# aromanro/DFTAtom

Measured on AMD Instinct MI355X. Metric: numerov_sweeps_per_s (executed sweeps of the reference's bisection path, whole SCF step; Rn Z=86 @ 131073 pts), higher is better.
Workload: dtype f64

## Files before the change

### dftatom_amd/__init__.py

```python
import ctypes as C
import os

import numpy as np

_HERE = os.path.dirname(os.path.abspath(__file__))
LIB_PATH = os.environ.get("DFTA_LIB_PATH") or os.path.join(_HERE, "libdftatom_hip.so")

OK = 0
SWEEP_COUNT, SWEEP_ZERO = 0, 1
SWEEP_KERNEL_AUTO, SWEEP_KERNEL_FUSED, SWEEP_KERNEL_PIPELINED = 0, 1, 2
BOUNDARY_DEVICE, BOUNDARY_HOST = 0, 1
LEVELS_CHAINED, LEVELS_BATCHED = 0, 1
LEVELS_SCAN_SWEEPS = 0x10
SWEEPS_EXACT, SWEEPS_TOLERANCE = 0, 1
ABI_VERSION = 7
LEVEL_CONVERGED, LEVEL_ITERATION_CAP, LEVEL_FIXED_POINT, LEVEL_U0_NONFINITE = 1, 2, 4, 8
POISSON_DEFAULT, POISSON_EXACT, POISSON_TOLERANCE, POISSON_ADAPTIVE = -1, 0, 1, 2
INT_TRAPEZOID, INT_SIMPSON13, INT_SIMPSON38, INT_BOOLE, INT_ROMBERG = range(5)
XC_VWN, XC_CHACHIYO, XC_CHACHIYO_IMPROVED, XC_PW92, XC_PBE = range(5)
AUFBAU_REFERENCE, AUFBAU_TRANSITION_METALS = range(2)
MIX_LINEAR, MIX_ANDERSON = range(2)
RECORD_DOUBLES = 64
ORB_PROPS = 8
ORB_NORM, ORB_RM1, ORB_R1, ORB_R2, ORB_R4, ORB_T, ORB_RPEAK, ORB_RM3 = range(8)
# ... 52 lines not shown
    "dfta_grid_destroy": (None, [vp]),
    "dfta_grid_num_nodes": (C.c_int, [vp]),
    "dfta_grid_rp": (C.c_double, [vp]),
    "dfta_grid_get_r": (C.c_int, [vp, c_dp]),
    "dfta_num_nodes": (C.c_int, [C.c_int]),
    "dfta_numerov_sweeps": (C.c_int, [vp, vp, C.c_int, C.c_int, C.c_int, c_dp, C.c_int, c_ip, c_ip, c_dp, c_ip,
                                      c_ip, c_dp, c_ip, c_ip]),
    "dfta_numerov_sweeps_scan": (C.c_int, [vp, vp, C.c_int, C.c_int, c_dp, C.c_int, c_ip, c_ip, c_dp, c_ip, c_ip, c_dp, c_ip, c_ip, c_ip]),
    "dfta_numerov_sweeps_dev": (C.c_int, [vp, vp, C.c_int, C.c_int, vp, C.c_int, c_ip, c_ip, c_ip, vp, vp, vp, vp, vp,
                                          vp, vp, vp, vp]),
    "dfta_numerov_match": (C.c_int, [vp, vp, C.c_int, C.c_int, c_dp, C.c_int, c_ip, c_ip, c_dp, c_dp, c_lp]),
    "dfta_potential_create": (C.c_int, [vp, vp, c_dp, C.POINTER(vp)]),
    "dfta_potential_update": (C.c_int, [vp, c_dp]),
    "dfta_potential_destroy": (None, [vp]),
    "dfta_potential_sweeps": (C.c_int, [vp, C.c_int, C.c_int, C.c_int, c_ip, c_dp, c_ip, c_ip, c_dp, c_ip, c_ip]),
    "dfta_potential_match": (C.c_int, [vp, C.c_int, c_ip, c_dp, c_dp, c_lp]),
    "dfta_solve_levels": (C.c_int, [vp, vp, C.c_int, C.c_int, C.c_int, c_dp, c_dp, c_dp, C.c_int, c_ip, c_ip, c_ip, c_ip,
                                    C.POINTER(LevelResult), c_dp, c_dp, c_dp, c_lp]),
    "dfta_poisson_create": (C.c_int, [vp, vp, C.c_int, C.POINTER(vp)]),
    "dfta_poisson_destroy": (None, [vp]),
    "dfta_poisson_solve": (C.c_int, [vp, c_ip, c_dp, c_dp, c_ip, c_dp]),
    "dfta_poisson_solve_dev": (C.c_int, [vp, vp, vp, vp]),
    "dfta_poisson_group_info": (C.c_int, [vp, c_ip, c_ip, c_ip]),
    "dfta_scf_poisson_info": (C.c_int, [vp, c_ip, c_ip, c_ip]),
    "dfta_poisson_level_size": (C.c_int, [vp, C.c_int]),
    "dfta_poisson_set_level": (C.c_int, [vp, C.c_int, c_dp, c_dp]),
    "dfta_poisson_get_level": (C.c_int, [vp, C.c_int, c_dp, c_dp]),
    "dfta_poisson_gauss_seidel": (C.c_int, [vp, C.c_int, C.c_int, c_dp]),
    "dfta_poisson_iterate_gs": (C.c_int, [vp, C.c_int, C.c_double, C.c_int, C.POINTER(C.c_double), C.POINTER(C.c_int)]),
    "dfta_poisson_restrict": (C.c_int, [vp, C.c_int]),
    "dfta_poisson_prolong": (C.c_int, [vp, C.c_int]),
    "dfta_poisson_vcycle": (C.c_int, [vp, c_dp]),
    "dfta_poisson_full_cycle": (C.c_int, [vp, C.c_double, C.c_double, C.c_double, C.c_double, c_dp, c_ip]),
    "dfta_scf_set_integrator": (C.c_int, [vp, C.c_int]),
    "dfta_vwn_lda": (C.c_int, [vp, c_dp, C.c_size_t, c_dp, c_dp]),
    "dfta_vwn_lsda": (C.c_int, [vp, c_dp, c_dp, C.c_size_t, c_dp, c_dp, c_dp, c_dp]),
    "dfta_integrate": (C.c_int, [vp, C.c_int, C.c_double, c_dp, C.c_int, C.POINTER(C.c_double)]),
    "dfta_scf_create": (C.c_int, [vp, vp, C.c_int, C.c_int, c_ip, C.c_double, C.c_int, C.c_int, C.POINTER(vp)]),
    "dfta_scf_create_ex": (C.c_int, [vp, vp, C.c_int, C.c_int, c_ip, C.c_double, C.c_int, C.c_int, vp, C.POINTER(vp)]),
    "dfta_scf_destroy": (None, [vp]),
    "dfta_scf_step": (C.c_int, [vp, C.POINTER(StepStats)]),
    "dfta_scf_get_energies": (C.c_int, [vp, C.POINTER(Energies), c_ip]),
    "dfta_scf_info": (C.c_int, [vp, c_ip, c_ip, c_lp]),
    "dfta_scf_num_levels": (C.c_int, [vp, C.c_int, C.c_int]),
    "dfta_scf_get_levels": (C.c_int, [vp, C.c_int, C.c_int, c_ip, c_ip, c_ip, c_dp, c_ip]),
    "dfta_scf_get_level_status": (C.c_int, [vp, C.c_int, C.c_int, c_ip, c_ip, c_ip]),
# ... 291 lines not shown
        self.ctx, self.grid, self.batch = ctx, grid, batch
        h = vp()
        if mode == POISSON_DEFAULT:
            ctx.check(ctx.lib.dfta_poisson_create(ctx.h, grid.h, batch, C.byref(h)))
        else:
            ctx.check(ctx.lib.dfta_poisson_create_ex(ctx.h, grid.h, batch, int(mode), C.byref(h)))
        self.h = h
        self.mode = ctx.lib.dfta_poisson_mode(h)

    def solve(self, Z, density):
        Z = _i32(np.atleast_1d(Z))
        rho = _f64(density).reshape(self.batch, self.grid.N)
        U = np.zeros_like(rho)
        vc = np.zeros(self.batch, np.int32)
        err = np.zeros(self.batch)
        self.ctx.check(self.ctx.lib.dfta_poisson_solve(self.h, _ip(Z), _dp(rho), _dp(U), _ip(vc), _dp(err)))
        return U, vc, err

    def group_info(self):
        g, d, a = C.c_int(), C.c_int(), C.c_int()
        self.ctx.check(self.ctx.lib.dfta_poisson_group_info(self.h, C.byref(g), C.byref(d), C.byref(a)))
        return g.value, bool(d.value), a.value

    def level_size(self, lvl):
        return self.ctx.lib.dfta_poisson_level_size(self.h, lvl)

    def set_level(self, lvl, phi=None, src=None):
        self.ctx.check(self.ctx.lib.dfta_poisson_set_level(self.h, lvl, _dp(_f64(phi)) if phi is not None else None,
                                                           _dp(_f64(src)) if src is not None else None))

    def get_level(self, lvl):
        n = self.level_size(lvl)
        phi, src = np.zeros(n), np.zeros(n)
        self.ctx.check(self.ctx.lib.dfta_poisson_get_level(self.h, lvl, _dp(phi), _dp(src)))
        return phi, src

    def gauss_seidel(self, lvl, sweeps=1):
        err = np.zeros(sweeps)
        self.ctx.check(self.ctx.lib.dfta_poisson_gauss_seidel(self.h, lvl, sweeps, _dp(err)))
        return err

    def iterate_gs(self, lvl, error_min, iterno):
        err = C.c_double()
        n = C.c_int()
        self.ctx.check(self.ctx.lib.dfta_poisson_iterate_gs(self.h, lvl, error_min, iterno, C.byref(err), C.byref(n)))
        return err.value, n.value
# ... 288 lines not shown
```

### dftatom_amd/csrc/poisson.hip

```cpp
#include <hip/hip_runtime.h>

#include <algorithm>
#include <cmath>
#include <cstdlib>
#include <memory>
#include <type_traits>
#include <vector>

#include "internal.h"
#include "poisson_plan.h"
#include "xc.h"

using namespace dfta_mg;

namespace {

#ifndef DFTA_KWARM
#define DFTA_KWARM 96
#endif
constexpr int kPF = 8;

__host__ __device__ __forceinline__ int addr(const Lvl& L, int i)
{
    if (i == L.n - 1) return L.n - 1;
// ... 168 lines not shown
    ++p->aborts;
    DFTA_HIP(ctx, hipMemsetAsync(p->d_total_vcycles, 0, sizeof(unsigned long long), ctx->stream));
    int rc = degrade(p);
    if (rc) return rc;
    rc = dfta_poisson_solve_launch(p->fallback.get(), dNe, dDensity, dU, dVcycles, dErr, dSkip);
    if (rc) return rc;
    DFTA_HIP(ctx, hipStreamSynchronize(ctx->stream));
    return DFTA_OK;
}

int dfta_poisson_take_vcycles(dfta_poisson* p, unsigned long long* out)
{
    dfta_ctx* ctx = p->ctx;
    unsigned long long a = 0, b = 0;
    DFTA_HIP(ctx, hipMemcpyAsync(&a, p->d_total_vcycles, sizeof(unsigned long long), hipMemcpyDeviceToHost, ctx->stream));
    if (p->fallback) DFTA_HIP(ctx, hipMemcpyAsync(&b, p->fallback->d_total_vcycles, sizeof(unsigned long long), hipMemcpyDeviceToHost, ctx->stream));
    DFTA_HIP(ctx, hipStreamSynchronize(ctx->stream));
    DFTA_HIP(ctx, hipMemsetAsync(p->d_total_vcycles, 0, sizeof(unsigned long long), ctx->stream));
    if (p->fallback) DFTA_HIP(ctx, hipMemsetAsync(p->fallback->d_total_vcycles, 0, sizeof(unsigned long long), ctx->stream));
    *out = a + b;
    return DFTA_OK;
}

int dfta_poisson_group_state(const dfta_poisson* p, int* G, int* degraded, int* aborts)
{
    if (!p) return DFTA_ERR_INVALID;
    if (G) *G = p->resident ? p->res_wg() : p->D.G;
    if (degraded) *degraded = p->degraded ? 1 : 0;
    if (aborts) *aborts = p->aborts;
    return DFTA_OK;
}

extern "C" {

int dfta_poisson_create_ex(dfta_ctx* ctx, const dfta_grid* g, int batch, int mode, dfta_poisson** out)
{
    if (!ctx || !g || !out) return DFTA_ERR_INVALID;
    DFTA_ENTER(ctx);
    DFTA_REQUIRE(ctx, mode == DFTA_POISSON_EXACT || mode == DFTA_POISSON_TOLERANCE || mode == DFTA_POISSON_ADAPTIVE, "poisson mode");
    return poisson_create_impl(ctx, g, batch, -1, mode, out);
}

int dfta_poisson_create(dfta_ctx* ctx, const dfta_grid* g, int batch, dfta_poisson** out)
{
    if (!ctx || !g || !out) return DFTA_ERR_INVALID;
    DFTA_ENTER(ctx);
// ... 9 lines not shown
    auto set = [](const char* value) { return value != nullptr; };
    auto on_off = [](const char* value) { return value ? (atoi(value) != 0 ? 1 : 0) : -1; };
    PoissonKnobs K;
    if (const char* e = dfta_knob("POISSON_GROUP")) {
        const int v = atoi(e);
        K.group_set = true;
        if (v >= 0 && v <= 6 && (batch << v) <= 256) K.group = v;
    }
    if (const char* e = dfta_knob("FAULT_POISSON_MEMBER")) K.fault = atoi(e) != 0;
    K.res = on_off(dfta_knob("POISSON_RES"));
    K.res16 = on_off(dfta_knob("POISSON_RES16"));
    K.nostage = set(dfta_knob("POISSON_NOSTAGE"));
    K.nostage_wave = set(dfta_knob("POISSON_NOSTAGE_WAVE"));
    K.nostage_shared = set(dfta_knob("POISSON_NOSTAGE_SHARED"));
    K.nocoarse = set(dfta_knob("POISSON_NOCOARSE"));
    K.noxw = set(dfta_knob("POISSON_NOXW"));
    K.norc = set(dfta_knob("POISSON_NORC"));
    K.nofuse3 = set(dfta_knob("POISSON_NOFUSE3"));
    K.nofuse3_wave = set(dfta_knob("POISSON_NOFUSE3_WAVE"));
    K.nohalf129 = set(dfta_knob("POISSON_NOHALF129"));
    K.nofold = set(dfta_knob("POISSON_NOFOLD"));
    K.nofold_lds = set(dfta_knob("POISSON_NOFOLD_LDS"));
    K.nofuse_coop = set(dfta_knob("POISSON_NOFUSE_COOP"));
    if (const char* e = dfta_knob("POISSON_FUSE_MIN_LOGC")) K.fuse_min_logc = std::max(kFuseMinLogC, atoi(e));
    if (const char* e = dfta_knob("POISSON_DBG")) K.dbg = atoi(e);
    K.plain_launch = set(dfta_knob("POISSON_PLAIN_LAUNCH")) || getenv("ROCP_TOOL_LIBRARIES") != nullptr;
    const char* m = dfta_knob("POISSON_MODE");
    K.mode = (m && m[0] == 't') ? DFTA_POISSON_TOLERANCE : ((m && m[0] == 'a') ? DFTA_POISSON_ADAPTIVE : DFTA_POISSON_EXACT);
    return K;
}

#define TRY_HIP(call) do { const hipError_t e_ = (call); if (e_ != hipSuccess) return e_; } while (0)
static hipError_t allocate(dfta_poisson* p)
{
    const PoissonPlan& P = *p;
    hipStream_t st = p->ctx->stream;
    TRY_HIP(p->d_phi0.alloc(P.n_level_store));
    TRY_HIP(p->d_phi1.alloc(P.n_level_store));
    TRY_HIP(p->d_src.alloc(P.n_level_store));
    TRY_HIP(p->d_cur.alloc(P.n_cur));
    TRY_HIP(p->d_desc.alloc(1));
    TRY_HIP(hipMemcpyAsync(p->d_desc, &p->D, sizeof(MgDesc), hipMemcpyHostToDevice, st));
    TRY_HIP(p->d_total_vcycles.alloc(1));
    TRY_HIP(p->d_group_ctr.alloc(P.n_group_ctr));
    TRY_HIP(p->d_group_part.alloc(P.n_group_part));
    TRY_HIP(p->d_res_slots.alloc(P.n_res_slots));
    TRY_HIP(p->d_res_spill.alloc(P.n_res_spill));
    TRY_HIP(hipMemsetAsync(p->d_phi0, 0, P.n_level_store * sizeof(double), st));
    TRY_HIP(hipMemsetAsync(p->d_phi1, 0, P.n_level_store * sizeof(double), st));
    TRY_HIP(hipMemsetAsync(p->d_src, 0, P.n_level_store * sizeof(double), st));
    TRY_HIP(hipMemsetAsync(p->d_cur, 0, P.n_cur * sizeof(int), st));
    TRY_HIP(hipMemsetAsync(p->d_total_vcycles, 0, sizeof(unsigned long long), st));
    return hipStreamSynchronize(st);
}
#undef TRY_HIP

static int blocks_per_cu(const void* kernel)
{
    int per_cu = 0;
    return hipOccupancyMaxActiveBlocksPerMultiprocessor(&per_cu, kernel, kThreads, 0) == hipSuccess ? per_cu : -1;
}

static int poisson_create_impl(dfta_ctx* ctx, const dfta_grid* g, int batch, int force_logG, int mode, dfta_poisson** out)
{
    DFTA_REQUIRE(ctx, batch >= 1 && g->levels <= kMaxLevels, "poisson batch/levels");
    PlanInputs in;
    in.knobs = read_knobs(batch);
    if (mode == kModeFromKnob) mode = in.knobs.mode;
    in.N = g->N; in.levels = g->levels; in.delta = g->delta; in.uniform = g->uniform;
    in.batch = batch; in.force_logG = force_logG; in.mode = mode; in.num_cu = ctx->num_cu;
    const bool tol = mode != DFTA_POISSON_EXACT;
    in.occupancy = [tol](PlanKernel k) {
        const KernelSet& K = kKernels[tol][k == kKernelSolveRes16];
        return blocks_per_cu(k == kKernelSolve ? reinterpret_cast<const void*>(K.solve) : reinterpret_cast<const void*>(K.solve_res));
    };
// ... 238 lines not shown
```

### dftatom_amd/csrc/poisson_kernels.inc

```
constexpr int kWarm = DFTA_MG_KWARM;
struct Atom {
    double* phi0;
    double* phi1;
    double* src;
    double* lds;
    double* stage;
    unsigned cur;
    int g, G;
    unsigned* ctr;
    unsigned bar;
    double* part;
    double* fslot;
    unsigned fseq;
    double* xchg;
    int pend;
    int pend_r;
    int pend_z;
    int lds_holds;
    int spin_max;
    bool gave_up;
    __device__ __forceinline__ int lane() const { return g * kThreads + static_cast<int>(threadIdx.x); }
    __device__ __forceinline__ double* cur_phi(int l, const Lvl& L) const
    {
        const unsigned c = (cur >> l) & 1u;
        return L.seq ? lds + c * kSeqCap + L.soff : (c ? phi1 : phi0) + L.off;
    }
    __device__ __forceinline__ double* other_phi(int l, const Lvl& L) const
    {
        const unsigned c = ((cur >> l) & 1u) ^ 1u;
        return L.seq ? lds + c * kSeqCap + L.soff : (c ? phi1 : phi0) + L.off;
    }
    __device__ __forceinline__ double* src_of(const Lvl& L) const { return L.seq ? lds + 2 * kSeqCap + L.soff : src + L.off; }
};

__device__ __forceinline__ void group_sync(Atom& A)
{
    if (A.G == 1) { __syncthreads(); return; }
    __syncthreads();
    ++A.bar;
    if (threadIdx.x == 0) {
        __builtin_amdgcn_fence(__ATOMIC_RELEASE, "agent");
        __hip_atomic_fetch_add(A.ctr, 1u, __ATOMIC_RELAXED, __HIP_MEMORY_SCOPE_AGENT);
        const unsigned target = A.bar * static_cast<unsigned>(A.G);
// ... 362 lines not shown
            for (int q = 0; q < kH; ++q) { bv[q] = ps[(r + kH + q) * RS]; bx[q] = pp[((r + kH + q + 1) & Cm1) * RS]; }
            __builtin_amdgcn_sched_barrier(0);
            own(ax, as, r);
            if (r + 2 * kH < C) {
#pragma unroll
                for (int q = 0; q < kH; ++q) { as[q] = ps[(r + 2 * kH + q) * RS]; ax[q] = pp[(r + 2 * kH + q + 1) * RS]; }
            }
            __builtin_amdgcn_sched_barrier(0);
            own(bx, bv, r + kH);
        }
    }
    if (lo_g == 0) pp[0] = node0;
    return err2;
}

constexpr int kWarm3 = DFTA_MG_KWARM3;
__device__ __forceinline__ double gs_point2y(double s, double y, double yp, double dh2)
{
    const double t1 = __builtin_fma(y, 0.5, s);
    const double u = yp - y;
    const double a = __builtin_fma(yp, 0.5, t1);
    return a - dh2 * u;
}
template <int LOGC, int RS, int NT, int KST, bool CAREFUL, bool RIGHT = false>
__device__ __forceinline__ void gs_lds3(const double* __restrict__ SSbase, double* __restrict__ PPbase, const int tid, const int lo_g,
                                        const bool last_lane, const double xN, const double dh, double& e1, double& e2, double& e3,
                                        const double* rightP = nullptr, const double* rightS = nullptr)
{
    constexpr int C = 1 << LOGC, Cm1 = C - 1, kH = 8, W = kWarm3;
    static_assert(C >= 4 && C <= 32 && W % (2 * kH) == 0, "fused pass: 4..32 nodes per lane");
    typedef __attribute__((address_space(3))) double lds_f64;
    typedef __attribute__((address_space(3))) const double lds_cf64;
    const bool active = tid < NT;
    lds_cf64* ps = (lds_cf64*)(SSbase) + tid;
    lds_f64* pp = (lds_f64*)(PPbase) + tid;
    asm volatile("" : "+v"(ps), "+v"(pp));
    auto off = [](int r) constexpr -> int { return (r & Cm1) * RS + (r >> LOGC); };
    const int neg_lo = -lo_g;
    const double dh2 = 0.5 * dh;
    const double Y0 = 2.0 * PPbase[0];
    double a1 = 0, a2 = 0, a3 = 0;
    double y1 = 0, y2 = 0, y3 = 0, sA = 0, sB = 0, o0 = 0, y1p = 0, y2p = 0;
    double xr0 = 0, xr1 = 0, xr2 = 0, sr0 = 0, sr1 = 0;
    double ax[kH], as[kH], bx[kH], bv[kH];
    auto load = [&](double (&X)[kH], double (&SV)[kH], const int r0) {
        const int col = r0 >> LOGC;
        if constexpr (C <= kH) {
            lds_cf64* bs = ps + col;
            lds_cf64* bp = (lds_cf64*)pp + col;
#pragma unroll
// ... 29 lines not shown
        constexpr int nq = C < kH ? C : kH;
        lds_f64* po = pp + r0 * RS;
#pragma unroll
        for (int q = 0; q < nq; ++q) {
            const double xn = (q == nq - 1) ? ((r0 + nq == C) ? xr0 : X[q]) : X[q];
            double t = gs_point2(SV[q], y1, xn, dh);
            if (CAREFUL && first && q == 0) t = (lo_g == 0) ? Y0 : t;
            { const double d = __builtin_fma(t, -0.5, o0); a1 = __builtin_fma(d, d, a1); }
            double u = gs_point2y(sA, y2, t, dh2);
            if (CAREFUL && first && q == 1) u = (lo_g == 0) ? Y0 : u;
            if (!(first && q == 0)) { const double d = y1p - u; a2 = __builtin_fma(d, d, a2); }
            double v = gs_point2y(sB, y3, u, dh2);
            if (CAREFUL && first && q == 2) v = (lo_g == 0) ? Y0 : v;
            if (!(first && q < 2)) { const double d = y2p - v; a3 = __builtin_fma(d, d, a3); }
            if (KST == 1) po[q * RS] = 0.5 * t;
            if (KST == 2 && !(first && q == 0)) po[(q - 1) * RS] = 0.5 * u;
            if (KST == 3 && !(first && q < 2)) po[(q - 2) * RS] = 0.5 * v;
            y1 = t; y2 = u; y3 = v;
            sB = sA; sA = SV[q];
            o0 = xn; y1p = t; y2p = u;
        }
    };
    if (active) {
        y1 = 2.0 * pp[off(-W - 1)]; y2 = 2.0 * pp[off(-W - 2)]; y3 = 2.0 * pp[off(-W - 3)];
        sA = ps[off(-W - 1)]; sB = ps[off(-W - 2)];
        load(ax, as, -W);
        for (int r0 = -W; r0 < 0; r0 += 2 * kH) {
            load(bx, bv, r0 + kH);
            __builtin_amdgcn_sched_barrier(0);
            warm(ax, as, r0);
            load(ax, as, r0 + 2 * kH);
            __builtin_amdgcn_sched_barrier(0);
            warm(bx, bv, r0 + kH);
        }
        y1p = y1; y2p = y2;
        xr0 = last_lane ? xN : pp[off(C)];
        xr1 = pp[off(C + 1)]; xr2 = pp[off(C + 2)];
        sr0 = ps[off(C)]; sr1 = ps[off(C + 1)];
        if (RIGHT && tid == NT - 1 && !last_lane) { xr0 = rightP[0]; xr1 = rightP[1]; xr2 = rightP[2]; sr0 = rightS[0]; sr1 = rightS[1]; }
    }
    if constexpr (NT <= 64) { __builtin_amdgcn_fence(__ATOMIC_SEQ_CST, "wavefront"); __builtin_amdgcn_wave_barrier(); }
    else __syncthreads();
    if (active) {
        if constexpr (C <= kH) {
            own(std::true_type{}, ax, as, 0);
        } else {
            for (int r0 = 0; r0 < C; r0 += 2 * kH) {
                load(bx, bv, r0 + kH);
                __builtin_amdgcn_sched_barrier(0);
                if (r0 == 0) own(std::true_type{}, ax, as, 0); else own(std::false_type{}, ax, as, r0);
                if (r0 + 2 * kH < C) load(ax, as, r0 + 2 * kH);
                __builtin_amdgcn_sched_barrier(0);
                own(std::false_type{}, bx, bv, r0 + kH);
            }
        }
        if (KST >= 2) {
            const double Y_N = 2.0 * xN;
            double t = gs_point2(sr0, y1, xr1, dh);
            t = last_lane ? Y_N : t;
            double u = gs_point2y(sA, y2, t, dh2);
            { const double d = y1p - u; a2 = __builtin_fma(d, d, a2); }
            if (KST == 2) pp[Cm1 * RS] = 0.5 * u;
            if (KST == 3) {
                double v = gs_point2y(sB, y3, u, dh2);
                { const double d = y2p - v; a3 = __builtin_fma(d, d, a3); }
                pp[(C - 2) * RS] = 0.5 * v;
                y1 = t; y2 = u; y3 = v; sB = sA; sA = sr0; y2p = u;
                t = gs_point2(sr1, y1, xr2, dh);
                u = gs_point2y(sA, y2, t, dh2);
                u = last_lane ? Y_N : u;
                v = gs_point2y(sB, y3, u, dh2);
                { const double d = y2p - v; a3 = __builtin_fma(d, d, a3); }
                pp[Cm1 * RS] = 0.5 * v;
            }
        }
    }
    e1 = a1; e2 = 0.25 * a2; e3 = 0.25 * a3;
}
// ... 432 lines not shown
            };
            int k0 = 0;
            for (; k0 + 16 <= C1; k0 += 16) rows(std::integral_constant<int, 16>{}, k0);
            for (; k0 + 8 <= C1; k0 += 8) rows(std::integral_constant<int, 8>{}, k0);
            for (; k0 < C1; k0 += 4) rows(std::integral_constant<int, 4>{}, k0);
            if (tid == 0) PP[L.n - 1] = G0[L.n - 1] + corr(L.n - 1, false);
        } else {
            copy_rows2(PP, SS, kThreads, G0, Sg, kThreads, C1);
            if (tid == 0) PP[L.n - 1] = G0[L.n - 1];
        }
        __syncthreads();
        PROF_ADD(5, l); };
        stage_in();
        const int lo_g = tid << L.logC;
        double err = 1E10;
        int done = 0;
        PROF_T0();
        bool fused_done = false;
        if (D.fuse3 && iterno == 3 && L.logC >= 2) {
            double f1, f2, f3;
            const bool lastl = tid == kThreads - 1;
            const double xN = PP[L.n - 1];
            const bool careful = (__builtin_amdgcn_readfirstlane(lo_g) <= kWarm3);
#define DFTA_GS3(LC) do { if (careful) gs_lds3<LC, kThreads, kThreads, 3, true>(SS, PP, tid, lo_g, lastl, xN, dh, f1, f2, f3); \
                          else gs_lds3<LC, kThreads, kThreads, 3, false>(SS, PP, tid, lo_g, lastl, xN, dh, f1, f2, f3); } while (0)
            switch (L.logC) {
                case 2:  DFTA_GS3(2); break;
                case 3:  DFTA_GS3(3); break;
                case 4:  DFTA_GS3(4); break;
                default: DFTA_GS3(5); break;
            }
#undef DFTA_GS3
            f1 = wave_total(f1); f2 = wave_total(f2); f3 = wave_total(f3);
            __syncthreads();
            if ((tid & 63) == 0) { red[tid >> 6] = f1; red[4 + (tid >> 6)] = f2; red[8 + (tid >> 6)] = f3; }
            __syncthreads();
            const double e1 = sqrt((red[0] + red[1]) + (red[2] + red[3]));
            const double e2 = sqrt((red[4] + red[5]) + (red[6] + red[7]));
            const double e3 = sqrt((red[8] + red[9]) + (red[10] + red[11]));
            if (!(e1 < errorMin) && !(e2 < errorMin)) {
                err = e3;
                done = 3;
                *nsweeps += 3;
                fused_done = true;
            } else {
                __syncthreads();
                stage_in();
            }
        }
        if (!fused_done)
        for (int i = 0; i < iterno; ++i) {
            double err2;
            switch (L.logC) {
                case 0:  err2 = gs_lds<0, kThreads>(SS, PP, tid, lo_g, dh); break;
                case 1:  err2 = gs_lds<1, kThreads>(SS, PP, tid, lo_g, dh); break;
                case 2:  err2 = gs_lds<2, kThreads>(SS, PP, tid, lo_g, dh); break;
                case 3:  err2 = gs_lds<3, kThreads>(SS, PP, tid, lo_g, dh); break;
                case 4:  err2 = gs_lds<4, kThreads>(SS, PP, tid, lo_g, dh); break;
                default: err2 = gs_lds<5, kThreads>(SS, PP, tid, lo_g, dh); break;
// ... 516 lines not shown
    lds_f64* P = (lds_f64*)(Pg);
    const int t = threadIdx.x & 63, i = t + 1;
    const bool mine = i < n - 1;
    const double a = 0.5 * (1.0 + dh), omd = 1.0 - dh;
    const double old = mine ? P[i] : 0.0;
    double c = mine ? 0.5 * __builtin_fma(omd, P[i + 1], S[i]) : 0.0;
    if (t == 0) c = __builtin_fma(a, P[0], c);
    wave_sync();
    double v = c, ratio = a;
#pragma unroll
    for (int off = 1; off < 64; off <<= 1) {
        const double up = __shfl_up(v, off, 64);
        if (t >= off) v = __builtin_fma(ratio, up, v);
        ratio *= ratio;
    }
    const double dif = old - v;
    if (mine) P[i] = v;
    return mine ? dif * dif : 0.0;
}
#endif

#ifndef DFTA_MG_SCAN_COARSE
template <int LOGC, int NT = 64>
__device__ __forceinline__ bool cs_visit3(const double* __restrict__ S, double* __restrict__ P, const double dh, const double errorMin, double& err)
{
    constexpr int C = 1 << LOGC;
    typedef __attribute__((address_space(3))) double lds_f64;
    lds_f64* pl = (lds_f64*)(P);
    const int lane = threadIdx.x & 63;
    double keep[C];
#pragma unroll
    for (int k = 0; k < C; ++k) keep[k] = pl[(k << 6) + lane];
    const double xN = pl[C << 6];
    double f1, f2, f3;
    gs_lds3<LOGC, 64, NT, 3, true>(S, P, lane, lane << LOGC, lane == NT - 1, xN, dh, f1, f2, f3);
    const double e1 = sqrt(wave_total(f1)), e2 = sqrt(wave_total(f2)), e3 = sqrt(wave_total(f3));
    wave_sync();
    if (!(e1 < errorMin) && !(e2 < errorMin)) { err = e3; return true; }
    if (lane < NT) {
#pragma unroll
        for (int k = 0; k < C; ++k) pl[(k << 6) + lane] = keep[k];
    }
    wave_sync();
    return false;
}
#endif

__device__ __forceinline__ double cs_iterate(const MgDesc& D, Atom& A, int l, double errorMin, int iterno, long* nsweeps)
{
    const Lvl L = D.lv[l];
    const double dh = L.d * 0.5;
    const int lane = threadIdx.x;
    double* P = A.stage + D.cs_phi[l];
    const double* S = A.stage + D.cs_src[l];
    const int lc = D.cs_lc[l];
    double err = 1E10;
#ifndef DFTA_MG_SCAN_COARSE
    const bool half = lc == 2 && L.n == 129;
    if (D.fuse3w && iterno == 3 && lc >= 2 && lc <= 4) {
        bool done;
        switch (lc) {
            case 2:  done = half ? cs_visit3<2, 32>(S, P, dh, errorMin, err) : cs_visit3<2>(S, P, dh, errorMin, err); break;
            case 3:  done = cs_visit3<3>(S, P, dh, errorMin, err); break;
            default: done = cs_visit3<4>(S, P, dh, errorMin, err); break;
        }
        if (done) { *nsweeps += 3; return err; }
    }
#else
    const bool half = false;
#endif
    for (int i = 0; i < iterno; ++i) {
        double err2 = 0;
#ifdef DFTA_MG_SCAN_COARSE
        if (lc >= 0) {
            switch (lc) {
                case 1:  err2 = cs_sweep_scan<1>(S, P, L.n, dh); break;
                case 2:  err2 = cs_sweep_scan<2>(S, P, L.n, dh); break;
                case 3:  err2 = cs_sweep_scan<3>(S, P, L.n, dh); break;
                default: err2 = cs_sweep_scan<4>(S, P, L.n, dh); break;
            }
            err2 = wave_total(err2);
        } else if (true) {
            err2 = cs_sweep_scan_small(S, P, L.n, dh);
            err2 = wave_total(err2);
        } else
#endif
        if (lc >= 0) {
// ... 1392 lines not shown
        res_init_coarse(D, A, R, rho, r, psrc, 0.0, Ne[a]);
    }
    const double err = res_cycles(D, A, R, 100, 1E-3, 1E-14, red, c);
    if (R.role == 0) {
        const Lvl L0 = D.lv[0];
        DFTA_RES_LEVEL(R.logC0, ({
            using Y = ResLay<LC>;
            const double* P = res_pp(R, 0);
            const int a0 = R.m * Y::N;
            for (int j = threadIdx.x; j < Y::N; j += kThreads) {
                const double v = P[Y::off(j)];
                U[(size_t)a * N + a0 + j] = v;
                A.phi0[L0.off + addr(L0, a0 + j)] = v;
            }
            if (R.m == kResG - 1 && threadIdx.x == 0) {
                const double v = P[Y::off(Y::N)];
                U[(size_t)a * N + N - 1] = v;
                A.phi0[L0.off + addr(L0, N - 1)] = v;
            }
        }))
    } else if (threadIdx.x == 0) {
        if (vcycles) vcycles[a] = (int)c.vcycles;
        if (errs) errs[a] = err;
        if (total_vcycles) atomicAdd(total_vcycles, (unsigned long long)c.vcycles);
    }
#ifdef DFTA_POISSON_RPROF
    __syncthreads();
    if (a == 0 && (R.role == 1 || R.m == 0) && threadIdx.x < 64) g_rprof[R.role * 64 + threadIdx.x] += prof_acc[threadIdx.x];
#endif
}

#ifndef DFTA_MG_RES16
__global__ __launch_bounds__(kThreads) void k_poisson_solve(const MgDesc* __restrict__ Dp, double* __restrict__ phi0, double* __restrict__ phi1,
                                                            double* __restrict__ src, const double* __restrict__ Ne,
                                                            const double* __restrict__ density, const double* __restrict__ r,
                                                            const double* __restrict__ psrc, double* __restrict__ U,
                                                            int* __restrict__ vcycles, double* __restrict__ errs,
                                                            unsigned long long* __restrict__ total_vcycles,
                                                            unsigned* __restrict__ group_ctr, double* __restrict__ group_part,
                                                            const int* __restrict__ skip, int fault, int src_all)
{
    __shared__ double red[20];
    __shared__ double seqmem[3 * kSeqCap];
    __shared__ double stagemem[2 * kStageArr];
    const MgDesc& D = *Dp;
    const int a = blockIdx.x >> D.logG;
    if (skip && skip[a]) return;
    if (fault && D.G > 1 && (blockIdx.x & (D.G - 1)) == D.G - 1) return;
    Atom A;
    A.phi0 = phi0 + (size_t)a * D.per_atom;
    A.phi1 = phi1 + (size_t)a * D.per_atom;
    A.src = src + (size_t)a * D.per_atom;
    A.lds = seqmem;
    A.stage = stagemem;
    A.cur = 0;
    A.G = D.G;
    A.g = blockIdx.x & (D.G - 1);
    A.ctr = group_ctr + a;
    A.bar = 0;
    A.part = group_part + (size_t)a * group_part_doubles(D.G);
    A.fslot = A.part + 6 * D.G + 2;
    A.xchg = A.part + (6 + kGrpBuf) * D.G + 2;
    A.fseq = 0;
    A.pend = 0;
    A.pend_r = 0;
// ... 5 lines not shown
    const int N = L0.n;
    const double* rho = density + (size_t)a * N;
    const bool coop0 = D.kcoop > 0;
    if (coop0 || A.g == 0)
    for (int idx = coop0 ? A.lane() : static_cast<int>(threadIdx.x); idx < N; idx += coop0 ? kThreads * A.G : kThreads) {
        const int i = node_of(L0, idx);
        double s = r[i];
        if (src_all || (i > 0 && i < N - 1)) s *= psrc[i] * rho[i];
        A.src[L0.off + idx] = s;
    }
    __syncthreads();
    Counters c{0, 0};
    PROF_T0();
    initialize(D, A, 0.0, Ne[a]);
    const double err = run_cycles<true>(D, A, 0, 100, 1E-3, 1E-14, red, c);
    PROF_ADD(5, 21);
    const double* __restrict__ P = A.cur_phi(0, L0);
    if (coop0 || A.g == 0)
        for (int i = coop0 ? A.lane() : static_cast<int>(threadIdx.x); i < N; i += coop0 ? kThreads * A.G : kThreads)
            U[(size_t)a * N + i] = P[addr(L0, i)];
    if (threadIdx.x == 0 && A.g == 0) {
        if (vcycles) vcycles[a] = (int)c.vcycles;
        if (errs) errs[a] = err;
        if (total_vcycles) atomicAdd(total_vcycles, (unsigned long long)c.vcycles);
    }
}

__global__ __launch_bounds__(kThreads) void k_unit(const MgDesc* __restrict__ Dp, double* phi0, double* phi1, double* src, int* cur, int op,
                                                   int lvl, int sweeps, double* out, unsigned* group_ctr, double* group_part)
{
    __shared__ double red[20];
    __shared__ double seqmem[3 * kSeqCap];
    __shared__ double stagemem[2 * kStageArr];
    const MgDesc& D = *Dp;
    Atom A;
    A.phi0 = phi0; A.phi1 = phi1; A.src = src; A.lds = seqmem;
    A.stage = stagemem;
    A.G = D.G;
    A.g = blockIdx.x;
    A.ctr = group_ctr;
    A.bar = 0;
    A.part = group_part;
    A.fslot = A.part + 6 * D.G + 2;
    A.xchg = A.part + (6 + kGrpBuf) * D.G + 2;
    A.fseq = 0;
    A.pend = 0;
    A.pend_r = 0;
    A.pend_z = 0;
    A.lds_holds = -1;
    A.spin_max = D.spin_max;
    A.gave_up = false;
    A.cur = 0;
    for (int l = 0; l < D.levels; ++l) A.cur |= (cur[l] ? 1u : 0u) << l;
    for (int l = 0; l < D.levels && A.g == 0; ++l) {
// ... 53 lines not shown
```

### dftatom_amd/csrc/poisson_plan.cpp

```cpp
#include "poisson_plan.h"

#include <algorithm>
#include <cmath>

namespace dfta_mg {
namespace {

int choose_group_size(const PlanInputs& in)
{
    const int batch = in.batch;
    int logG = batch <= 16 ? 4 : (batch <= 32 ? 3 : (batch <= 64 ? 2 : ((batch <= 128 && 2 * batch <= std::max(in.num_cu, 1)) ? 1 : 0)));
    if (batch <= 4 && in.N - 1 >= (1 << 20)) logG = 5;
    if (in.knobs.group >= 0) logG = in.knobs.group;
    if (in.force_logG >= 0) logG = in.force_logG;
    return logG;
}

void choose_resident(const PlanInputs& in, PoissonPlan& P)
{
    const PoissonKnobs& K = in.knobs;
    const int batch = in.batch;
    const bool free_choice = in.force_logG < 0 && !K.nostage;
    bool want = batch * kResWG <= in.num_cu && free_choice && !K.group_set;
    if (K.res >= 0) want = K.res != 0 && free_choice && batch * kResWG <= 256;
// ... 145 lines not shown

}

int plan_poisson(const PlanInputs& in, PoissonPlan* plan)
{
    *plan = PoissonPlan();
    PoissonPlan& P = *plan;
    MgDesc& D = P.D;
    const PoissonKnobs& K = in.knobs;
    D.levels = in.levels;
    P.tol = in.mode == 1 || in.mode == 2;
    P.adaptive = in.mode == 2;
    P.fault = K.fault;
    P.plain_launch = K.plain_launch;
    D.spin_max = P.fault ? (1 << 12) : (1 << 23);
    int logG = choose_group_size(in);
    choose_resident(in, P);
    D.logG = fit_to_occupancy(in, P, logG);
    D.G = 1 << D.logG;
    D.nofold = K.nofold ? 1 : 0;
    D.fold_lds = K.nofold_lds ? 0 : 1;
    D.fuse3 = K.nofuse3 ? 0 : 1;
    D.fuse3w = (D.fuse3 && !K.nofuse3_wave) ? 1 : 0;
    D.fuse_min_logc = K.fuse_min_logc;
    D.fuse_coop = K.nofuse_coop ? 0 : 1;
    D.dbg = K.dbg;
    D.adaptive = P.adaptive ? 1 : 0;
    P.seq_doubles = lay_out_levels(in, D);
    classify_staging(K, D);
    plan_coarse_section(K, P.tol, D);
    plan_xw(K, P.tol, D);
    plan_rc(K, P.tol, D);
    if (P.seq_doubles > kSeqCap) { P.error = "sequential levels exceed LDS budget"; return 1; }
    count_allocations(in, P);
    return 0;
}

}
```

### dftatom_amd/csrc/poisson_plan.h

```cpp
#pragma once

#include <cstddef>
#include <functional>

#if defined(__HIPCC__)
#define DFTA_MG_HD __host__ __device__
#else
#define DFTA_MG_HD
#endif

namespace dfta_mg {

constexpr int kMaxLevels = 24;
constexpr int kThreads = 256;
constexpr int kSeqBelow = 129;
constexpr int kWaveMaxN = 1025;
constexpr int kSeqCap = 144;
constexpr int kFuseMinLogC = 6;
constexpr int kStageMaxLogC = 5;
constexpr int kStagePad = 128;
constexpr int kStageH = 24;
constexpr int kStageRS = kThreads + kStageH;
constexpr int kStageArr = 8992;
constexpr int kPad = 320;
constexpr int kWarm3Exact = 112, kWarm3Tol = 32;

struct Lvl {
    int n;
    int logC;
    int logT;
    int seq;
    int stage;
    long off;
    long soff;
    double d;
};

struct MgDesc {
    int levels;
    int G;
    int logG;
    int dbg;
    int res_kres;
    int res_logC0;
    int fuse_min_logc;
    int fuse_coop;
    int fuse3;
    int fuse3w;
    int nofold;
    int fold_lds;
    int kcoop;
    int spin_max;
    long per_atom;
    int cs_top;
    int xw_top;
    int rc_src[6];
    int adaptive;
    int rc_top;
    int cs_phi[kMaxLevels], cs_src[kMaxLevels], cs_lc[kMaxLevels];
    Lvl lv[kMaxLevels];
};

constexpr int kXchg = 128;
constexpr unsigned kGrpBuf = 8;
DFTA_MG_HD constexpr size_t group_part_doubles(int G) { return (size_t)(6 + kGrpBuf) * G + 2 + (size_t)kGrpBuf * G * kXchg; }

constexpr int kResNT = 128;
constexpr int kResG = 32;
constexpr int kResWG = kResG + 1;
constexpr int kRes16NT = 256, kRes16G = 16, kRes16WG = kRes16G + 1;
constexpr int kResX = 272;
constexpr int kResMaxShared = 4;
constexpr int kResXTail = 0, kResXSrc = 128, kResXHead = 256, kResXS0 = 266;
constexpr unsigned kResBuf = 16;
DFTA_MG_HD constexpr size_t res_slot_doubles() { return (size_t)kResBuf * kResWG * 4 + (size_t)kResBuf * kResWG * kResX; }

struct PoissonKnobs {
    bool group_set = false;
    int group = -1;
    int res = -1, res16 = -1;
    bool nostage = false, nostage_wave = false, nostage_shared = false;
    bool nocoarse = false, noxw = false, norc = false;
    bool nofuse3 = false, nofuse3_wave = false, nohalf129 = false;
    bool nofold = false, nofold_lds = false, nofuse_coop = false;
    int fuse_min_logc = kFuseMinLogC;
    int dbg = 0;
    bool plain_launch = false;
    int fault = 0;
    int mode = 0;
};

enum PlanKernel { kKernelSolve, kKernelSolveRes, kKernelSolveRes16 };

struct PlanInputs {
    int N = 0, levels = 0;
    double delta = 0;
    int uniform = 0;
    int batch = 1;
    int force_logG = -1;
    int mode = 0;
    int num_cu = 0;
    std::function<int(PlanKernel)> occupancy;
    PoissonKnobs knobs;
};

struct PoissonPlan {
    MgDesc D = {};
// ... 22 lines not shown
```

### include/dftatom_hip.h

```cpp
#ifndef DFTATOM_HIP_H
#define DFTATOM_HIP_H

#include <stddef.h>
#include <stdint.h>

#ifdef __cplusplus
extern "C" {
#endif

#define DFTA_OK              0
#define DFTA_ERR_INVALID     1
#define DFTA_ERR_NO_DEVICE   2
#define DFTA_ERR_HIP         3
#define DFTA_ERR_NOMEM       4
#define DFTA_ERR_NOT_CONVERGED 5

typedef struct dfta_ctx     dfta_ctx;
typedef struct dfta_grid    dfta_grid;
typedef struct dfta_poisson dfta_poisson;
typedef struct dfta_scf     dfta_scf;

int         dfta_ctx_create(int device, void* hip_stream, dfta_ctx** out);
void        dfta_ctx_destroy(dfta_ctx* ctx);
int         dfta_ctx_synchronize(dfta_ctx* ctx);
// ... 73 lines not shown
#define DFTA_LEVEL_U0_NONFINITE  8

int dfta_solve_levels(dfta_ctx* ctx, const dfta_grid* g, int mode, int tree_depth,
                      int nV, const double* V, const double* bottom0 ,
                      const double* bottom_hint ,
                      int nlevels, const int* vidx, const int* n, const int* l, const int* occ,
                      dfta_level_result* results,
                      double* newDensity ,
                      double* Eelectronic ,
                      double* Psi_out ,
                      long* issued_sweeps );

int  dfta_poisson_create(dfta_ctx* ctx, const dfta_grid* g, int batch, dfta_poisson** out);
#define DFTA_POISSON_EXACT     0
#define DFTA_POISSON_TOLERANCE 1
#define DFTA_POISSON_ADAPTIVE 2
int  dfta_poisson_create_ex(dfta_ctx* ctx, const dfta_grid* g, int batch, int mode, dfta_poisson** out);
int  dfta_poisson_mode(const dfta_poisson* p);
void dfta_poisson_destroy(dfta_poisson* p);
int  dfta_poisson_solve(dfta_poisson* p, const int* Z, const double* density, double* U,
                        int* vcycles_out, double* err_out);
int  dfta_poisson_solve_dev(dfta_poisson* p, const int* dZ, const double* dDensity, double* dU);
int  dfta_poisson_group_info(const dfta_poisson* p, int* G, int* degraded, int* aborts);
int  dfta_poisson_level_size(const dfta_poisson* p, int lvl);
int  dfta_poisson_set_level(dfta_poisson* p, int lvl, const double* Phi, const double* Src);
int  dfta_poisson_get_level(dfta_poisson* p, int lvl, double* Phi, double* Src);
int  dfta_poisson_gauss_seidel(dfta_poisson* p, int lvl, int sweeps, double* err_out );
int  dfta_poisson_iterate_gs(dfta_poisson* p, int lvl, double errorMin, int iterno, double* err_out, int* sweeps_out);
int  dfta_poisson_restrict(dfta_poisson* p, int lvl);
int  dfta_poisson_prolong(dfta_poisson* p, int lvl_src);
int  dfta_poisson_vcycle(dfta_poisson* p, double* err_out);
int  dfta_poisson_full_cycle(dfta_poisson* p, double lowBoundary, double highBoundary, double errorMin, double errorMinLast,
                             double* err_out, int* vcycles_out);

int dfta_vwn_lda(dfta_ctx* ctx, const double* n, size_t sz, double* vexc, double* eexcdif);
int dfta_vwn_lsda(dfta_ctx* ctx, const double* na, const double* nb, size_t sz,
                  double* vexc, double* va, double* vb, double* eexcdif);

int dfta_chachiyo_lda(dfta_ctx* ctx, int improved, const double* n, size_t sz, double* vexc, double* eexcdif);

int dfta_xc_pointwise(dfta_ctx* ctx, int functional, size_t sz, const double* na, const double* nb,
                      const double* saa, const double* sab, const double* sbb,
                      double* e, double* dna, double* dnb, double* dsaa, double* dsab, double* dsbb);
int dfta_xc_radial(dfta_ctx* ctx, const dfta_grid* g, int functional, int natoms, const double* na, const double* nb,
                   double* res, double* va, double* vb, double* eexc);

// ... 116 lines not shown
```

Before: 39270.

## Shorten Gauss-Seidel warmup in fused 3-sweep passes with bitwise handoff check and redo

The fused three-sweep Gauss-Seidel passes (wave-level coarse visit and the staged LDS path) now start with a shorter warmup window (88 instead of the full exact window) by default in exact mode. After each shortened pass, every lane compares the three carried values it received against its left neighbour's outputs, across waves via shared memory. If any differ bitwise, the staged data is restored and the pass reruns with the full warmup, so results stay exact. This trims redundant warmup recomputation at the cost of extra comparison, barrier and reduction work, possible redo passes, larger shared reduction arrays, and new counters plus a query API.

```diff
diff --git a/dftatom_amd/__init__.py b/dftatom_amd/__init__.py
--- a/dftatom_amd/__init__.py
+++ b/dftatom_amd/__init__.py
@@ -98,6 +98,7 @@
     "dfta_poisson_solve": (C.c_int, [vp, c_ip, c_dp, c_dp, c_ip, c_dp]),
     "dfta_poisson_solve_dev": (C.c_int, [vp, vp, vp, vp]),
     "dfta_poisson_group_info": (C.c_int, [vp, c_ip, c_ip, c_ip]),
+    "dfta_poisson_take_short_warmups": (C.c_int, [vp, C.POINTER(C.c_ulonglong), C.POINTER(C.c_ulonglong)]),
     "dfta_scf_poisson_info": (C.c_int, [vp, c_ip, c_ip, c_ip]),
     "dfta_poisson_level_size": (C.c_int, [vp, C.c_int]),
     "dfta_poisson_set_level": (C.c_int, [vp, C.c_int, c_dp, c_dp]),
@@ -435,6 +436,11 @@
         self.ctx.check(self.ctx.lib.dfta_poisson_group_info(self.h, C.byref(g), C.byref(d), C.byref(a)))
         return g.value, bool(d.value), a.value
 
+    def take_short_warmups(self):
+        v, r = C.c_ulonglong(), C.c_ulonglong()
+        self.ctx.check(self.ctx.lib.dfta_poisson_take_short_warmups(self.h, C.byref(v), C.byref(r)))
+        return v.value, r.value
+
     def level_size(self, lvl):
         return self.ctx.lib.dfta_poisson_level_size(self.h, lvl)
 
diff --git a/dftatom_amd/csrc/poisson.hip b/dftatom_amd/csrc/poisson.hip
--- a/dftatom_amd/csrc/poisson.hip
+++ b/dftatom_amd/csrc/poisson.hip
@@ -214,6 +214,21 @@
     return DFTA_OK;
 }
 
+int dfta_poisson_take_short_warmups(dfta_poisson* p, unsigned long long* visits, unsigned long long* redos)
+{
+    if (!p) return DFTA_ERR_INVALID;
+    dfta_ctx* ctx = p->ctx;
+    unsigned long long a[2] = {0, 0}, b[2] = {0, 0};
+    DFTA_HIP(ctx, hipMemcpyAsync(a, p->d_total_vcycles + 1, sizeof(a), hipMemcpyDeviceToHost, ctx->stream));
+    if (p->fallback) DFTA_HIP(ctx, hipMemcpyAsync(b, p->fallback->d_total_vcycles + 1, sizeof(b), hipMemcpyDeviceToHost, ctx->stream));
+    DFTA_HIP(ctx, hipStreamSynchronize(ctx->stream));
+    DFTA_HIP(ctx, hipMemsetAsync(p->d_total_vcycles + 1, 0, sizeof(a), ctx->stream));
+    if (p->fallback) DFTA_HIP(ctx, hipMemsetAsync(p->fallback->d_total_vcycles + 1, 0, sizeof(b), ctx->stream));
+    if (redos) *redos = a[0] + b[0];
+    if (visits) *visits = a[1] + b[1];
+    return DFTA_OK;
+}
+
 int dfta_poisson_group_state(const dfta_poisson* p, int* G, int* degraded, int* aborts)
 {
     if (!p) return DFTA_ERR_INVALID;
@@ -269,6 +284,9 @@
     K.nofold = set(dfta_knob("POISSON_NOFOLD"));
     K.nofold_lds = set(dfta_knob("POISSON_NOFOLD_LDS"));
     K.nofuse_coop = set(dfta_knob("POISSON_NOFUSE_COOP"));
+    K.noshortwarm_wave = set(dfta_knob("POISSON_NOSHORTWARM_WAVE"));
+    K.noshortwarm_stage = set(dfta_knob("POISSON_NOSHORTWARM_STAGE"));
+    if (const char* e = dfta_knob("POISSON_SHORTWARM")) K.shortwarm = atoi(e);
     if (const char* e = dfta_knob("POISSON_FUSE_MIN_LOGC")) K.fuse_min_logc = std::max(kFuseMinLogC, atoi(e));
     if (const char* e = dfta_knob("POISSON_DBG")) K.dbg = atoi(e);
     K.plain_launch = set(dfta_knob("POISSON_PLAIN_LAUNCH")) || getenv("ROCP_TOOL_LIBRARIES") != nullptr;
@@ -288,7 +306,7 @@
     TRY_HIP(p->d_cur.alloc(P.n_cur));
     TRY_HIP(p->d_desc.alloc(1));
     TRY_HIP(hipMemcpyAsync(p->d_desc, &p->D, sizeof(MgDesc), hipMemcpyHostToDevice, st));
-    TRY_HIP(p->d_total_vcycles.alloc(1));
+    TRY_HIP(p->d_total_vcycles.alloc(3));
     TRY_HIP(p->d_group_ctr.alloc(P.n_group_ctr));
     TRY_HIP(p->d_group_part.alloc(P.n_group_part));
     TRY_HIP(p->d_res_slots.alloc(P.n_res_slots));
@@ -297,7 +315,7 @@
     TRY_HIP(hipMemsetAsync(p->d_phi1, 0, P.n_level_store * sizeof(double), st));
     TRY_HIP(hipMemsetAsync(p->d_src, 0, P.n_level_store * sizeof(double), st));
     TRY_HIP(hipMemsetAsync(p->d_cur, 0, P.n_cur * sizeof(int), st));
-    TRY_HIP(hipMemsetAsync(p->d_total_vcycles, 0, sizeof(unsigned long long), st));
+    TRY_HIP(hipMemsetAsync(p->d_total_vcycles, 0, 3 * sizeof(unsigned long long), st));
     return hipStreamSynchronize(st);
 }
 #undef TRY_HIP
diff --git a/dftatom_amd/csrc/poisson_kernels.inc b/dftatom_amd/csrc/poisson_kernels.inc
--- a/dftatom_amd/csrc/poisson_kernels.inc
+++ b/dftatom_amd/csrc/poisson_kernels.inc
@@ -19,6 +19,7 @@
     int lds_holds;
     int spin_max;
     bool gave_up;
+    unsigned sw_visits = 0, sw_redos = 0;
     __device__ __forceinline__ int lane() const { return g * kThreads + static_cast<int>(threadIdx.x); }
     __device__ __forceinline__ double* cur_phi(int l, const Lvl& L) const
     {
@@ -427,10 +428,12 @@
     const double a = __builtin_fma(yp, 0.5, t1);
     return a - dh2 * u;
 }
+struct Hand3 { double in[3], out[3]; };
 template <int LOGC, int RS, int NT, int KST, bool CAREFUL, bool RIGHT = false>
 __device__ __forceinline__ void gs_lds3(const double* __restrict__ SSbase, double* __restrict__ PPbase, const int tid, const int lo_g,
                                         const bool last_lane, const double xN, const double dh, double& e1, double& e2, double& e3,
-                                        const double* rightP = nullptr, const double* rightS = nullptr)
+                                        const double* rightP = nullptr, const double* rightS = nullptr, const int w = kWarm3,
+                                        Hand3* hand = nullptr)
 {
     constexpr int C = 1 << LOGC, Cm1 = C - 1, kH = 8, W = kWarm3;
     static_assert(C >= 4 && C <= 32 && W % (2 * kH) == 0, "fused pass: 4..32 nodes per lane");
@@ -506,10 +509,19 @@
         }
     };
     if (active) {
-        y1 = 2.0 * pp[off(-W - 1)]; y2 = 2.0 * pp[off(-W - 2)]; y3 = 2.0 * pp[off(-W - 3)];
-        sA = ps[off(-W - 1)]; sB = ps[off(-W - 2)];
-        load(ax, as, -W);
+        y1 = 2.0 * pp[off(-w - 1)]; y2 = 2.0 * pp[off(-w - 2)]; y3 = 2.0 * pp[off(-w - 3)];
+        sA = ps[off(-w - 1)]; sB = ps[off(-w - 2)];
+        const int first = -(w & ~kH);
+        if (w & kH) {
+            load(bx, bv, -w);
+            load(ax, as, first);
+            __builtin_amdgcn_sched_barrier(0);
+            warm(bx, bv, -w);
+        } else {
+            load(ax, as, first);
+        }
         for (int r0 = -W; r0 < 0; r0 += 2 * kH) {
+            if (r0 < first) continue;
             load(bx, bv, r0 + kH);
             __builtin_amdgcn_sched_barrier(0);
             warm(ax, as, r0);
@@ -518,6 +530,7 @@
             warm(bx, bv, r0 + kH);
         }
         y1p = y1; y2p = y2;
+        if (hand) { hand->in[0] = y1; hand->in[1] = y2; hand->in[2] = y3; }
         xr0 = last_lane ? xN : pp[off(C)];
         xr1 = pp[off(C + 1)]; xr2 = pp[off(C + 2)];
         sr0 = ps[off(C)]; sr1 = ps[off(C + 1)];
@@ -538,6 +551,7 @@
                 own(std::false_type{}, bx, bv, r0 + kH);
             }
         }
+        if (hand) { hand->out[0] = y1; hand->out[1] = y2; hand->out[2] = y3; }
         if (KST >= 2) {
             const double Y_N = 2.0 * xN;
             double t = gs_point2(sr0, y1, xr1, dh);
@@ -1016,19 +1030,48 @@
             const bool lastl = tid == kThreads - 1;
             const double xN = PP[L.n - 1];
             const bool careful = (__builtin_amdgcn_readfirstlane(lo_g) <= kWarm3);
-#define DFTA_GS3(LC) do { if (careful) gs_lds3<LC, kThreads, kThreads, 3, true>(SS, PP, tid, lo_g, lastl, xN, dh, f1, f2, f3); \
-                          else gs_lds3<LC, kThreads, kThreads, 3, false>(SS, PP, tid, lo_g, lastl, xN, dh, f1, f2, f3); } while (0)
-            switch (L.logC) {
-                case 2:  DFTA_GS3(2); break;
-                case 3:  DFTA_GS3(3); break;
-                case 4:  DFTA_GS3(4); break;
-                default: DFTA_GS3(5); break;
-            }
+            auto pass = [&](const int w, Hand3* h) -> bool {
+#define DFTA_GS3(LC) do { if (careful) gs_lds3<LC, kThreads, kThreads, 3, true>(SS, PP, tid, lo_g, lastl, xN, dh, f1, f2, f3, nullptr, nullptr, w, h); \
+                          else gs_lds3<LC, kThreads, kThreads, 3, false>(SS, PP, tid, lo_g, lastl, xN, dh, f1, f2, f3, nullptr, nullptr, w, h); } while (0)
+                switch (L.logC) {
+                    case 2:  DFTA_GS3(2); break;
+                    case 3:  DFTA_GS3(3); break;
+                    case 4:  DFTA_GS3(4); break;
+                    default: DFTA_GS3(5); break;
+                }
 #undef DFTA_GS3
-            f1 = wave_total(f1); f2 = wave_total(f2); f3 = wave_total(f3);
-            __syncthreads();
-            if ((tid & 63) == 0) { red[tid >> 6] = f1; red[4 + (tid >> 6)] = f2; red[8 + (tid >> 6)] = f3; }
-            __syncthreads();
+                bool bad = false;
+                if (h) {
+                    if ((tid & 63) == 63 && tid != kThreads - 1) { double* z = red + 12 + 3 * (tid >> 6); z[0] = h->out[0]; z[1] = h->out[1]; z[2] = h->out[2]; }
+#pragma unroll
+                    for (int k = 0; k < 3; ++k)
+                        bad |= __builtin_bit_cast(long long, wt_dpp<0x138, 0xf>(h->out[k])) != __builtin_bit_cast(long long, h->in[k]);
+                    bad = bad && (tid & 63) != 0;
+                }
+                f1 = wave_total(f1); f2 = wave_total(f2); f3 = wave_total(f3);
+                __syncthreads();
+                if (h && (tid & 63) == 0 && tid != 0) {
+                    const double* z = red + 12 + 3 * ((tid >> 6) - 1);
+#pragma unroll
+                    for (int k = 0; k < 3; ++k) bad |= __builtin_bit_cast(long long, z[k]) != __builtin_bit_cast(long long, h->in[k]);
+                }
+                const bool wave_bad = h && __builtin_amdgcn_ballot_w64(bad) != 0;
+                if ((tid & 63) == 0) { red[tid >> 6] = f1; red[4 + (tid >> 6)] = f2; red[8 + (tid >> 6)] = f3; red[21 + (tid >> 6)] = wave_bad ? 1.0 : 0.0; }
+                __syncthreads();
+                return red[21] + red[22] + red[23] + red[24] == 0.0;
+            };
+            int w = (D.sw_stage > 0 && D.sw_stage < kWarm3) ? D.sw_stage : kWarm3;
+            for (;;) {
+                Hand3 h = {};
+                const bool passed = pass(w, w == kWarm3 ? nullptr : &h);
+                if (w == kWarm3) break;
+                ++A.sw_visits;
+                if (passed) break;
+                ++A.sw_redos;
+                __syncthreads();
+                stage_in();
+                w = kWarm3;
+            }
             const double e1 = sqrt((red[0] + red[1]) + (red[2] + red[3]));
             const double e2 = sqrt((red[4] + red[5]) + (red[6] + red[7]));
             const double e3 = sqrt((red[8] + red[9]) + (red[10] + red[11]));
@@ -1591,7 +1634,8 @@
 
 #ifndef DFTA_MG_SCAN_COARSE
 template <int LOGC, int NT = 64>
-__device__ __forceinline__ bool cs_visit3(const double* __restrict__ S, double* __restrict__ P, const double dh, const double errorMin, double& err)
+__device__ __forceinline__ bool cs_visit3(Atom& A, const double* __restrict__ S, double* __restrict__ P, const double dh, const double errorMin,
+                                          const int short_w, double& err)
 {
     constexpr int C = 1 << LOGC;
     typedef __attribute__((address_space(3))) double lds_f64;
@@ -1602,7 +1646,27 @@
     for (int k = 0; k < C; ++k) keep[k] = pl[(k << 6) + lane];
     const double xN = pl[C << 6];
     double f1, f2, f3;
-    gs_lds3<LOGC, 64, NT, 3, true>(S, P, lane, lane << LOGC, lane == NT - 1, xN, dh, f1, f2, f3);
+    int w = (short_w > 0 && short_w < kWarm3) ? short_w : kWarm3;
+    for (;;) {
+        Hand3 h = {};
+        gs_lds3<LOGC, 64, NT, 3, true>(S, P, lane, lane << LOGC, lane == NT - 1, xN, dh, f1, f2, f3, nullptr, nullptr, w, &h);
+        if (w == kWarm3) break;
+        ++A.sw_visits;
+        bool bad = false;
+#pragma unroll
+        for (int k = 0; k < 3; ++k)
+            bad |= __builtin_bit_cast(long long, wt_dpp<0x138, 0xf>(h.out[k])) != __builtin_bit_cast(long long, h.in[k]);
+        bad = bad && lane >= 1 && lane < NT;
+        if (__builtin_amdgcn_ballot_w64(bad) == 0) break;
+        ++A.sw_redos;
+        wave_sync();
+        if (lane < NT) {
+#pragma unroll
+            for (int k = 0; k < C; ++k) pl[(k << 6) + lane] = keep[k];
+        }
+        wave_sync();
+        w = kWarm3;
+    }
     const double e1 = sqrt(wave_total(f1)), e2 = sqrt(wave_total(f2)), e3 = sqrt(wave_total(f3));
     wave_sync();
     if (!(e1 < errorMin) && !(e2 < errorMin)) { err = e3; return true; }
@@ -1629,9 +1693,9 @@
     if (D.fuse3w && iterno == 3 && lc >= 2 && lc <= 4) {
         bool done;
         switch (lc) {
-            case 2:  done = half ? cs_visit3<2, 32>(S, P, dh, errorMin, err) : cs_visit3<2>(S, P, dh, errorMin, err); break;
-            case 3:  done = cs_visit3<3>(S, P, dh, errorMin, err); break;
-            default: done = cs_visit3<4>(S, P, dh, errorMin, err); break;
+            case 2:  done = half ? cs_visit3<2, 32>(A, S, P, dh, errorMin, D.sw_wave, err) : cs_visit3<2>(A, S, P, dh, errorMin, D.sw_wave, err); break;
+            case 3:  done = cs_visit3<3>(A, S, P, dh, errorMin, D.sw_wave, err); break;
+            default: done = cs_visit3<4>(A, S, P, dh, errorMin, D.sw_wave, err); break;
         }
         if (done) { *nsweeps += 3; return err; }
     }
@@ -3070,7 +3134,10 @@
     } else if (threadIdx.x == 0) {
         if (vcycles) vcycles[a] = (int)c.vcycles;
         if (errs) errs[a] = err;
-        if (total_vcycles) atomicAdd(total_vcycles, (unsigned long long)c.vcycles);
+        if (total_vcycles) {
+            atomicAdd(total_vcycles, (unsigned long long)c.vcycles);
+            if (A.sw_visits) { atomicAdd(total_vcycles + 1, (unsigned long long)A.sw_redos); atomicAdd(total_vcycles + 2, (unsigned long long)A.sw_visits); }
+        }
     }
 #ifdef DFTA_POISSON_RPROF
     __syncthreads();
@@ -3088,7 +3155,7 @@
                                                             unsigned* __restrict__ group_ctr, double* __restrict__ group_part,
                                                             const int* __restrict__ skip, int fault, int src_all)
 {
-    __shared__ double red[20];
+    __shared__ double red[32];
     __shared__ double seqmem[3 * kSeqCap];
     __shared__ double stagemem[2 * kStageArr];
     const MgDesc& D = *Dp;
@@ -3140,14 +3207,17 @@
     if (threadIdx.x == 0 && A.g == 0) {
         if (vcycles) vcycles[a] = (int)c.vcycles;
         if (errs) errs[a] = err;
-        if (total_vcycles) atomicAdd(total_vcycles, (unsigned long long)c.vcycles);
+        if (total_vcycles) {
+            atomicAdd(total_vcycles, (unsigned long long)c.vcycles);
+            if (A.sw_visits) { atomicAdd(total_vcycles + 1, (unsigned long long)A.sw_redos); atomicAdd(total_vcycles + 2, (unsigned long long)A.sw_visits); }
+        }
     }
 }
 
 __global__ __launch_bounds__(kThreads) void k_unit(const MgDesc* __restrict__ Dp, double* phi0, double* phi1, double* src, int* cur, int op,
                                                    int lvl, int sweeps, double* out, unsigned* group_ctr, double* group_part)
 {
-    __shared__ double red[20];
+    __shared__ double red[32];
     __shared__ double seqmem[3 * kSeqCap];
     __shared__ double stagemem[2 * kStageArr];
     const MgDesc& D = *Dp;
diff --git a/dftatom_amd/csrc/poisson_plan.cpp b/dftatom_amd/csrc/poisson_plan.cpp
--- a/dftatom_amd/csrc/poisson_plan.cpp
+++ b/dftatom_amd/csrc/poisson_plan.cpp
@@ -191,6 +191,11 @@
     D.fold_lds = K.nofold_lds ? 0 : 1;
     D.fuse3 = K.nofuse3 ? 0 : 1;
     D.fuse3w = (D.fuse3 && !K.nofuse3_wave) ? 1 : 0;
+    {
+        const int forced = K.shortwarm > 0 ? std::min(std::max(K.shortwarm / 8 * 8, 8), kWarm3Exact) : 0;
+        D.sw_wave = (P.tol || K.noshortwarm_wave) ? 0 : (forced ? forced : kShortWarmWave);
+        D.sw_stage = (P.tol || K.noshortwarm_stage) ? 0 : (forced ? forced : kShortWarmStage);
+    }
     D.fuse_min_logc = K.fuse_min_logc;
     D.fuse_coop = K.nofuse_coop ? 0 : 1;
     D.dbg = K.dbg;
diff --git a/dftatom_amd/csrc/poisson_plan.h b/dftatom_amd/csrc/poisson_plan.h
--- a/dftatom_amd/csrc/poisson_plan.h
+++ b/dftatom_amd/csrc/poisson_plan.h
@@ -24,6 +24,7 @@
 constexpr int kStageArr = 8992;
 constexpr int kPad = 320;
 constexpr int kWarm3Exact = 112, kWarm3Tol = 32;
+constexpr int kShortWarmWave = 88, kShortWarmStage = 88;
 
 struct Lvl {
     int n;
@@ -47,6 +48,8 @@
     int fuse_coop;
     int fuse3;
     int fuse3w;
+    int sw_wave;
+    int sw_stage;
     int nofold;
     int fold_lds;
     int kcoop;
@@ -83,6 +86,8 @@
     bool nocoarse = false, noxw = false, norc = false;
     bool nofuse3 = false, nofuse3_wave = false, nohalf129 = false;
     bool nofold = false, nofold_lds = false, nofuse_coop = false;
+    bool noshortwarm_wave = false, noshortwarm_stage = false;
+    int shortwarm = 0;
     int fuse_min_logc = kFuseMinLogC;
     int dbg = 0;
     bool plain_launch = false;
diff --git a/include/dftatom_hip.h b/include/dftatom_hip.h
--- a/include/dftatom_hip.h
+++ b/include/dftatom_hip.h
@@ -119,6 +119,7 @@
                         int* vcycles_out, double* err_out);
 int  dfta_poisson_solve_dev(dfta_poisson* p, const int* dZ, const double* dDensity, double* dU);
 int  dfta_poisson_group_info(const dfta_poisson* p, int* G, int* degraded, int* aborts);
+int  dfta_poisson_take_short_warmups(dfta_poisson* p, unsigned long long* visits, unsigned long long* redos);
 int  dfta_poisson_level_size(const dfta_poisson* p, int lvl);
 int  dfta_poisson_set_level(dfta_poisson* p, int lvl, const double* Phi, const double* Src);
 int  dfta_poisson_get_level(dfta_poisson* p, int lvl, double* Phi, double* Src);
```

After: 38850. -1.1%, worse.
